# PalamaraLab/FastSMC

Hardware: AMD Instinct MI355X
Metric: haplotype-pairs decoded/sec (whole node) + GB/s vs HBM roofline, 69-state HMM (higher is better)
Workload: dtype f32; 1 GPU; synthetic 1000 haplotypes x 50000 sites, K=69, all 499500 pairs per GPU, FastSMC-mode IBD + posterior-mean/MAP ages, no hashing; mode=ibd, resident_waves=2048, n_cu=256, chunk_sites=512, chunks_per_window=98, resident_chunks=24, beta_stride=2, kernel_member=69, record_gather=none, lib_hash=6c32ac588c314776

## Files before the change

### fastsmc_amd/csrc/fsmc_capi.hip

```cpp
#include <hip/hip_runtime.h>

#include <algorithm>
#include <chrono>
#include <cmath>
#include <cstdio>
#include <cstdlib>
#include <cstring>
#include <new>
#include <string>
#include <type_traits>
#include <vector>

#include "fsmc_identify.h"
#include "fsmc_instances.h"
#include "fsmc_pair_bins.h"
#include "fsmc_pair_cdf.h"
#include "fsmc_pair_tail.h"
#include "fsmc_pair_minima.h"
#include "fsmc_pair_posteriors.h"

namespace fsmc
{
hipError_t idSortCandidates(hipStream_t stream, const fsmc_candidate* in, fsmc_candidate* sorted, unsigned n,
                            unsigned nHaps, unsigned nWords);
hipError_t idSeedDepths(hipStream_t stream, const unsigned long long* words, unsigned nHaps, unsigned nWords,
                        unsigned maxSeeds, unsigned readAhead, unsigned char* depthOut,
                        unsigned hapStride);
}

using namespace fsmc;

namespace fsmc
{
__global__ void add_planes_in_order_kernel(const float* __restrict__ planes, float* __restrict__ acc, size_t n,
                                           int nPlanes, size_t planeStride)
{
  for (size_t i = (size_t)blockIdx.x * blockDim.x + threadIdx.x; i < n; i += (size_t)gridDim.x * blockDim.x) {
    float s = acc[i];
    for (int sl = 0; sl < nPlanes; ++sl) {
      s = s + planes[(size_t)sl * planeStride + i];
    }
    acc[i] = s;
  }
}
}

namespace
{
thread_local std::string g_createError;

struct DevBuf {
  void* p = nullptr;
  size_t bytes = 0;
};

constexpr int kChunkPoolDefault = -1;
constexpr uint32_t kChunkPoolPhiDefault = 200;

enum PairSlicing {
  kSlicePosteriors,
  kSliceMinima,
  kSliceBins,
  kSliceCdf,
  kSliceTail,
  kSliceLoglik,
  kSliceViterbi,
  kPairSlicings
};
}

struct fsmc_ctx {
  int device = 0;
  hipStream_t stream = nullptr;
  bool ownStream = false;
  int nCU = 0;
  uint64_t hbmBytes = 0;
  uint64_t wsLimit = 0;
  double wsEarned = 0;
  double wsAnnounced = 0;
  double wsAnnouncedCredit = 0;
  std::string err;

  unsigned long long* dHaps = nullptr;
  uint32_t nHaps = 0, nSites = 0, W = 0;

  fsmc_pair* dPairs = nullptr;
  fsmc_group* dGroups = nullptr;
  size_t nPairs = 0, nGroups = 0;
  std::vector<fsmc_pair> hPairs;
  std::vector<fsmc_group> hGroups;

  unsigned* dCounters = nullptr;
  unsigned long long* dPhase = nullptr;
  DevBuf ws;
  DevBuf recs;
  size_t recCap = 0;
  DevBuf aux;
  DevBuf out;

  hipEvent_t ev0 = nullptr, ev1 = nullptr;
  bool timed = false;
  int lastSlots = 0;
  int lastChunk = 0, lastMaxChunks = 0, lastResident = 0;
  int residentChunks = -1;
  int chunkPool = kChunkPoolDefault;
  uint32_t chunkPoolPhi = kChunkPoolPhiDefault;
  DevBuf poolState;
  uint32_t lastPoolBuffers = 0;
  uint32_t chunkSites = 0;
  uint32_t betaStride = 0;
  int lastStride = 1;
  bool lastSpsLds = false;
  int lastMember = 0;

  struct IbdQueues {
    uint64_t serial = 0;
    uint64_t maxLen = 0;
    uint64_t maxLenAlone = 0;
    uint32_t pairing = 0;
    bool valid = false;
    bool dual = false;
    bool reordered = false;
    bool alone = false;
    std::vector<fsmc_group> items, unions, rest;
  } q;
  uint64_t worklistSerial = 0;
  fsmc_group* dItems = nullptr;
  fsmc_group* dRest = nullptr;
  uint32_t pairing = 1;
  int lastItems = 0;
  unsigned twoWaves = 0;
  int lastWavesPerWindow = 1;
  hipStream_t side = nullptr;
  hipEvent_t evFork = nullptr, evJoin = nullptr;
  DevBuf wsSide;

  struct {
    uint32_t groups = 0;
    int last = 0;
  } pairSlices[kPairSlicings];
  DevBuf ppStage;
  DevBuf ppRows;
  DevBuf ppAcc;
  hipStream_t copyStream = nullptr;
  void* ppPinned[2] = {nullptr, nullptr};
  size_t ppPinnedBytes = 0;
  hipEvent_t evRows = nullptr, evCopied[2] = {nullptr, nullptr};
  DevBuf pmAcc;
  DevBuf pbAcc;
  DevBuf pcSpec;
  DevBuf plAcc;
  DevBuf pvAcc;
  DevBuf ptAcc;

  DevBuf idStash;
  size_t idStashCount = 0;

  const fsmc_model* ibdModel = nullptr;
  uint32_t ibdFlags = 0;
  bool ibdPending = false;
};

struct fsmc_model {
  fsmc_ctx* ctx = nullptr;
  int K = 0, KP = 0, S = 0, nRows = 0;
  int w2NW = 0;
  float *pi = nullptr, *cR = nullptr, *expT = nullptr;
  float *D = nullptr, *B = nullptr, *U = nullptr, *RR = nullptr;
  float* rowSets = nullptr;
  float* ghostMask = nullptr;
  int* stepRow = nullptr;
  bool sequence = false;
  int *rowGapF = nullptr, *rowSiteB = nullptr, *rowGapB = nullptr;
  float4* emis3 = nullptr;
  unsigned stateThr = 0, ageThr = 0;
  float probThr = 0.f;
};

namespace
{

std::vector<std::string> mappedHipRuntimes()
{
  std::vector<std::string> found;
  if (FILE* f = std::fopen("/proc/self/maps", "r")) {
    char line[4096];
    while (std::fgets(line, sizeof(line), f)) {
      const char* slash = std::strchr(line, '/');
      if (!slash || !std::strstr(slash, "libamdhip64.so")) {
        continue;
// ... 563 lines not shown
    if (ctx->chunkSites) {
      cMin = std::min<size_t>(ctx->chunkSites, L);
    }
    slots = std::min<size_t>(slots, (size_t)(budget.hard / slotBytes(cMin)));
    if (slots == 0) {
      why = "workspace limit too small for the back-pointers of one wave";
      return FSMC_ENOMEM;
    }
    if (ctx->chunkSites) {
      C = cMin;
    } else {
      const uint64_t room = L <= 512 ? budget.hard : budget.soft;
      while (C > cMin && (uint64_t)slots * slotBytes(C) > room) {
        C = std::max(cMin, (C + 1) / 2);
      }
    }
    bytes = slotBytes(C);
  }
  plan = LaunchPlan();
  plan.k = k;
  plan.chunk = (int)C;
  plan.chunkRows = (int)C;
  plan.maxChunks = (int)((L + C - 1) / C);
  plan.wsSlot = bytes / sizeof(float4);
  plan.slots = (int)slots;
  plan.wavesPerWindow = 1;
  plan.bytes = bytes * slots;
  return FSMC_OK;
}

bool twoWavesWanted(const fsmc_ctx* ctx, const KernelChoice& k2, size_t nItems)
{
  if (ctx->twoWaves == 1 || nItems == 0 || !k2.fn) {
    return false;
  }
  if (const char* v = std::getenv("FSMC_DIAG_TWO_WAVE_WINDOWS")) {
    if (std::strcmp(v, "never") == 0) {
      return false;
    }
  }
  int perCU = 0;
  return workgroupsPerCU(k2, 4, 2, perCU) == hipSuccess && perCU >= 1 && nItems <= (size_t)ctx->nCU * perCU;
}

bool planTwoWaves(const fsmc_ctx* ctx, const KernelChoice& k2, size_t nItems, const WsBudget& budget, LaunchPlan& plan)
{
  size_t L = 1;
  for (const fsmc_group& g : ctx->hGroups) {
    L = std::max<size_t>(L, g.to - g.from);
  }
  const size_t K4 = (size_t)(k2.member + 3) / 4;
  plan = LaunchPlan();
  plan.k = k2;
  plan.chunk = (int)L;
  plan.chunkRows = (int)L;
  plan.maxChunks = 1;
  plan.wsSlot = L * K4 * kWave;
  plan.slots = (int)nItems;
  plan.wavesPerWindow = 2;
  plan.bytes = plan.wsSlot * sizeof(float4) * nItems;
  return plan.bytes <= budget.hard && (plan.bytes <= budget.soft || L <= 512);
}

int holdWorkspace(fsmc_ctx* ctx, DevBuf& buf, size_t bytes)
{
  const char* most = std::getenv("FSMC_DIAG_WS_ALLOC_MAX");
  if (most && bytes > std::strtoull(most, nullptr, 10) && !(buf.p && buf.bytes >= bytes)) {
    if (buf.p) {
      (void)hipFree(buf.p);
    }
    buf = DevBuf();
    return fail(ctx, FSMC_ENOMEM, "workspace of " + std::to_string(bytes) + " bytes refused (FSMC_DIAG_WS_ALLOC_MAX)");
  }
  const size_t held = buf.bytes;
  const int rc = ensure(ctx, buf, bytes);
  if (rc != FSMC_OK) {
    (void)hipGetLastError();
  } else if (buf.bytes != held) {
    payForWorkspace(ctx, buf.bytes);
  }
  return rc;
}

int planAndHold(fsmc_ctx* ctx, const fsmc_model* m, int mode, const KernelChoice& k, const std::vector<fsmc_group>& list,
                bool paired, unsigned share, DevBuf& buf, LaunchPlan& plan)
{
  std::string why;
  const int rc = planOneWave(ctx, m, mode, k, list, paired, workspaceBudget(ctx, buf), share, plan, why);
  if (rc != FSMC_OK) {
    return fail(ctx, rc, why);
  }
  if (plan.poolBuffers) {
    FSMC_TRY(ensure(ctx, ctx->poolState, (kPoolClaims + (size_t)plan.poolBuffers) * sizeof(unsigned)));
  }
  return holdWorkspace(ctx, buf, plan.bytes);
}

void recordLaunch(fsmc_ctx* ctx, const KernelChoice& k, const LaunchPlan& plan, int slotsBeside = 0)
{
  ctx->lastMember = k.member;
  ctx->lastStride = k.stride;
  ctx->lastChunk = plan.chunk;
  ctx->lastMaxChunks = plan.maxChunks;
  ctx->lastResident = plan.residentChunks;
  ctx->lastPoolBuffers = plan.poolBuffers;
  ctx->lastWavesPerWindow = plan.wavesPerWindow;
  ctx->lastSlots = plan.slots + slotsBeside;
}

int checkReady(fsmc_ctx* ctx, const fsmc_model* m)
{
  if (!ctx || !m) {
    return fail(ctx, FSMC_EINVAL, "null context or model");
  }
  if (m->ctx != ctx) {
    return fail(ctx, FSMC_EINVAL, "model belongs to another context");
  }
  if (!ctx->dHaps) {
    return fail(ctx, FSMC_ESTATE, "no haplotypes uploaded (fsmc_haps_upload)");
  }
  if (!ctx->dPairs || !ctx->dGroups || ctx->nGroups == 0) {
    return fail(ctx, FSMC_ESTATE, "no work list uploaded (fsmc_worklist_upload)");
  }
  if ((uint32_t)m->S != ctx->nSites) {
    return fail(ctx, FSMC_EINVAL, "model has " + std::to_string(m->S) + " sites but haplotypes have " +
                                      std::to_string(ctx->nSites));
  }
  for (const fsmc_pair& pr : ctx->hPairs) {
    if (pr.hap_a >= ctx->nHaps || pr.hap_b >= ctx->nHaps) {
      return fail(ctx, FSMC_EINVAL, "pair refers to a haplotype row outside the uploaded matrix");
    }
  }
  for (const fsmc_group& g : ctx->hGroups) {
    if (g.to > (uint32_t)m->S) {
      return fail(ctx, FSMC_EINVAL, "group window exceeds the number of sites");
    }
  }
  if (m->K > kMaxStatesAny) {
    return fail(ctx, FSMC_EUNSUPPORTED, "more than " + std::to_string(kMaxStatesAny) + " states");
  }
  return FSMC_OK;
}

void fillParams(const fsmc_ctx* ctx, const fsmc_model* m, const LaunchPlan& plan, uint32_t flags, KParams& p)
{
  std::memset(&p, 0, sizeof(p));
  p.K = m->K;
  p.KP = m->KP;
  p.S = m->S;
  p.W = (int)ctx->W;
  p.nGroups = (int)ctx->nGroups;
  p.chunk = plan.chunk;
  p.chunkRows = plan.chunkRows;
  p.maxChunks = plan.maxChunks;
  p.residentChunks = plan.residentChunks;
  p.flags = flags;
  p.pi = m->pi;
  p.cR = m->cR;
  p.expT = m->expT;
  p.D = m->D;
  p.B = m->B;
  p.U = m->U;
  p.rowSets = m->rowSets;
  p.RR = m->RR;
  p.ghostMask = m->ghostMask;
  p.stepRow = m->stepRow;
  p.rowGapF = m->rowGapF;
  p.rowSiteB = m->rowSiteB;
  p.rowGapB = m->rowGapB;
  p.emis3 = m->emis3;
  p.haps = ctx->dHaps;
  p.pairs = ctx->dPairs;
  p.groups = ctx->dGroups;
  p.counters = ctx->dCounters;
  p.phaseCycles = ctx->dPhase;
  p.ws = (float4*)ctx->ws.p;
  p.wsSlot = plan.wsSlot;
  p.stateThr = m->stateThr;
  p.ageThr = m->ageThr;
  p.spsLds = 0u;
  p.thr[0] = 1000 * m->probThr;
  p.thr[1] = 100 * m->probThr;
  p.thr[2] = 10 * m->probThr;
  p.thr[3] = m->probThr;
  p.recs = (fsmc_ibd_record*)ctx->recs.p;
  p.recCap = (unsigned)ctx->recCap;
}

int checkWorkspace(fsmc_ctx* ctx, const KParams& p, int slots)
{
  const DevBuf& buf = p.ws == (float4*)ctx->wsSide.p ? ctx->wsSide : ctx->ws;
  if (!p.ws || p.ws != (float4*)buf.p || slots < 1 || buf.bytes / sizeof(float4) / (size_t)slots < p.wsSlot) {
    return fail(ctx, FSMC_ESTATE, "the workspace does not hold the launch planned for it");
  }
  return FSMC_OK;
}

int poolParams(fsmc_ctx* ctx, const KernelChoice& k, const KParams& p, const LaunchPlan& plan, int slots, KParamsPool& pp)
{
  static_cast<KParams&>(pp) = p;
  pp.poolOff = plan.poolOff;
  pp.poolBuffers = plan.poolBuffers;
  pp.poolCap = plan.poolCap;
  pp.poolState = (unsigned*)ctx->poolState.p;
  const DevBuf& buf = p.ws == (float4*)ctx->wsSide.p ? ctx->wsSide : ctx->ws;
  const size_t rowF4 = (size_t)((p.K + 3) / 4) * kWave;
  const size_t poolF4 = (size_t)pp.poolBuffers * (size_t)p.chunkRows * rowF4;
  if (!k.poolFn || pp.poolOff < p.wsSlot * (size_t)slots || buf.bytes / sizeof(float4) < pp.poolOff ||
      buf.bytes / sizeof(float4) - pp.poolOff < poolF4 || !pp.poolState ||
      ctx->poolState.bytes / sizeof(unsigned) < kPoolClaims + (size_t)pp.poolBuffers || pp.poolCap < 1 ||
      pp.poolCap > p.maxChunks) {
    return fail(ctx, FSMC_ESTATE, "the workspace does not hold the chunk pool planned for it");
  }
  return FSMC_OK;
}

int resetPool(fsmc_ctx* ctx, const KParamsPool& pp)
{
  FSMC_HIP(ctx, hipMemsetAsync(pp.poolState, 0, (kPoolClaims + (size_t)pp.poolBuffers) * sizeof(unsigned), ctx->stream));
  return FSMC_OK;
}

int launch(fsmc_ctx* ctx, const KernelChoice& k, const KParams& p, int slots, size_t dynLds = 0, bool continues = false,
           const LaunchPlan* plan = nullptr)
{
  if (checkWorkspace(ctx, p, slots) != FSMC_OK) {
    return FSMC_ESTATE;
  }
  const bool pool = plan && plan->poolBuffers != 0;
  KParamsPool pp;
  if (pool) {
    FSMC_TRY(poolParams(ctx, k, p, *plan, slots, pp));
  }
  FSMC_HIP(ctx, hipMemsetAsync(ctx->dCounters, 0, 4 * sizeof(unsigned), ctx->stream));
  if (pool) {
    FSMC_TRY(resetPool(ctx, pp));
  }
  if (!continues) {
    FSMC_HIP(ctx, hipEventRecord(ctx->ev0, ctx->stream));
  }
  if (pool) {
    hipLaunchKernelGGL(k.poolFn, dim3((unsigned)slots), dim3(k.threads), dynLds, ctx->stream, pp);
  } else {
    hipLaunchKernelGGL(k.fn, dim3((unsigned)slots), dim3(k.threads), dynLds, ctx->stream, p);
  }
  FSMC_HIP(ctx, hipGetLastError());
  FSMC_HIP(ctx, hipEventRecord(ctx->ev1, ctx->stream));
  ctx->timed = true;
  return FSMC_OK;
}

int launchBeside(fsmc_ctx* ctx, const KernelChoice& kSide, KParams& pSide, int slotsSide, const LaunchPlan& planSide,
                 const KernelChoice& kMain, KParams& pMain, int slotsMain)
{
  if (checkWorkspace(ctx, pSide, slotsSide) != FSMC_OK || checkWorkspace(ctx, pMain, slotsMain) != FSMC_OK) {
    return FSMC_ESTATE;
  }
  pMain.groupBase = 0;
  pSide.groupBase = 2;
  const bool pool = planSide.poolBuffers != 0;
  KParamsPool ppSide;
  if (pool) {
    FSMC_TRY(poolParams(ctx, kSide, pSide, planSide, slotsSide, ppSide));
  }
  FSMC_HIP(ctx, hipMemsetAsync(ctx->dCounters, 0, 4 * sizeof(unsigned), ctx->stream));
  if (pool) {
    FSMC_TRY(resetPool(ctx, ppSide));
  }
  FSMC_HIP(ctx, hipEventRecord(ctx->ev0, ctx->stream));
  FSMC_HIP(ctx, hipEventRecord(ctx->evFork, ctx->stream));
  FSMC_HIP(ctx, hipStreamWaitEvent(ctx->side, ctx->evFork, 0));
  if (pool) {
    hipLaunchKernelGGL(kSide.poolFn, dim3((unsigned)slotsSide), dim3(kSide.threads), 0, ctx->side, ppSide);
  } else {
    hipLaunchKernelGGL(kSide.fn, dim3((unsigned)slotsSide), dim3(kSide.threads), 0, ctx->side, pSide);
  }
  FSMC_HIP(ctx, hipGetLastError());
  hipLaunchKernelGGL(kMain.fn, dim3((unsigned)slotsMain), dim3(kMain.threads), 0, ctx->stream, pMain);
  FSMC_HIP(ctx, hipGetLastError());
  FSMC_HIP(ctx, hipEventRecord(ctx->evJoin, ctx->side));
  FSMC_HIP(ctx, hipStreamWaitEvent(ctx->stream, ctx->evJoin, 0));
  FSMC_HIP(ctx, hipEventRecord(ctx->ev1, ctx->stream));
  ctx->timed = true;
  return FSMC_OK;
}

uint64_t stagingLimit(const fsmc_ctx* ctx, uint64_t held, unsigned parts)
{
  uint64_t limit = ctx->wsLimit ? ctx->wsLimit : (uint64_t)(0.25 * (double)ctx->hbmBytes);
  size_t freeB = 0, totalB = 0;
  if (hipMemGetInfo(&freeB, &totalB) == hipSuccess) {
    const uint64_t room = (uint64_t)freeB + held;
    const uint64_t reserve = 2ull << 30;
    limit = std::min<uint64_t>(limit, room > reserve ? (room - reserve) / parts : 0);
  }
  return limit;
}

int ensureRowCopies(fsmc_ctx* ctx, size_t need)
{
  if (ctx->ppPinnedBytes < need) {
    for (int i = 0; i < 2; ++i) {
// ... 322 lines not shown
  }
  fsmc_ctx* ctx = new (std::nothrow) fsmc_ctx();
  if (!ctx) {
    return fail(nullptr, FSMC_ENOMEM, "host allocation failed");
  }
  ctx->device = device_id;
  e = hipSetDevice(device_id);
  hipDeviceProp_t prop;
  if (e == hipSuccess) {
    e = hipGetDeviceProperties(&prop, device_id);
  }
  if (e != hipSuccess) {
    delete ctx;
    return fail(nullptr, FSMC_ENODEVICE, std::string("hipSetDevice/hipGetDeviceProperties: ") + hipGetErrorString(e));
  }
  if (std::strncmp(prop.gcnArchName, "gfx950", 6) != 0) {
    std::string arch = prop.gcnArchName;
    delete ctx;
    return fail(nullptr, FSMC_ENODEVICE, "device is " + arch + "; this library is built for gfx950 (MI355X) only");
  }
  ctx->nCU = prop.multiProcessorCount;
  ctx->hbmBytes = (uint64_t)prop.totalGlobalMem;
  if (stream) {
    ctx->stream = (hipStream_t)stream;
  } else {
    e = hipStreamCreateWithFlags(&ctx->stream, hipStreamNonBlocking);
    ctx->ownStream = (e == hipSuccess);
  }
  if (e == hipSuccess) e = hipEventCreate(&ctx->ev0);
  if (e == hipSuccess) e = hipEventCreate(&ctx->ev1);
  if (e == hipSuccess) e = hipStreamCreateWithFlags(&ctx->side, hipStreamNonBlocking);
  if (e == hipSuccess) e = hipEventCreateWithFlags(&ctx->evFork, hipEventDisableTiming);
  if (e == hipSuccess) e = hipEventCreateWithFlags(&ctx->evJoin, hipEventDisableTiming);
  if (e == hipSuccess) e = hipMalloc((void**)&ctx->dCounters, 4 * sizeof(unsigned));
  if (e == hipSuccess) e = hipMalloc((void**)&ctx->dPhase, kPhaseSlots * sizeof(unsigned long long));
  if (e == hipSuccess) e = hipMemset(ctx->dPhase, 0, kPhaseSlots * sizeof(unsigned long long));
  if (e != hipSuccess) {
    std::string msg = std::string("context set-up failed: ") + hipGetErrorString(e);
    fsmc_ctx_destroy(ctx);
    return fail(nullptr, FSMC_EHIP, msg);
  }
  {
    int blocks = 0;
    const hipError_t pe = hipOccupancyMaxActiveBlocksPerMultiprocessor(
      &blocks, decode_kernel<128, kModeIbd, true, false, false>, kWave, 0);
    if (pe != hipSuccess) {
      (void)hipGetLastError();
      const std::vector<std::string> rts = mappedHipRuntimes();
      std::string msg = std::string("kernels of this library cannot be launched (") + hipGetErrorString(pe) + ")";
      int code = FSMC_EHIP;
      if (rts.size() > 1) {
        code = FSMC_ERUNTIME;
        msg += ": two HIP runtimes are loaded in this process (";
        for (size_t i = 0; i < rts.size(); ++i) {
          msg += (i ? ", " : "") + rts[i];
        }
        msg += "): load one libamdhip64 only -- e.g. import torch before this library so that both resolve to the "
               "copy torch bundles, or link both against the same ROCm";
      }
      fsmc_ctx_destroy(ctx);
      return fail(nullptr, code, msg);
    }
  }
  *out = ctx;
  return FSMC_OK;
}

void fsmc_ctx_destroy(fsmc_ctx* ctx)
{
  if (!ctx) {
    return;
  }
  (void)hipSetDevice(ctx->device);
  if (ctx->stream) {
    (void)hipStreamSynchronize(ctx->stream);
  }
  if (ctx->dHaps) (void)hipFree(ctx->dHaps);
  if (ctx->dPairs) (void)hipFree(ctx->dPairs);
  if (ctx->dGroups) (void)hipFree(ctx->dGroups);
  if (ctx->dItems) (void)hipFree(ctx->dItems);
  if (ctx->dRest) (void)hipFree(ctx->dRest);
  if (ctx->dCounters) (void)hipFree(ctx->dCounters);
  if (ctx->poolState.p) (void)hipFree(ctx->poolState.p);
  if (ctx->dPhase) (void)hipFree(ctx->dPhase);
  if (ctx->idStash.p) (void)hipFree(ctx->idStash.p);
  if (ctx->ws.p) (void)hipFree(ctx->ws.p);
  if (ctx->recs.p) (void)hipFree(ctx->recs.p);
  if (ctx->aux.p) (void)hipFree(ctx->aux.p);
  if (ctx->out.p) (void)hipFree(ctx->out.p);
  if (ctx->ev0) (void)hipEventDestroy(ctx->ev0);
  if (ctx->ev1) (void)hipEventDestroy(ctx->ev1);
  if (ctx->evFork) (void)hipEventDestroy(ctx->evFork);
  if (ctx->evJoin) (void)hipEventDestroy(ctx->evJoin);
  if (ctx->side) (void)hipStreamDestroy(ctx->side);
  if (ctx->wsSide.p) (void)hipFree(ctx->wsSide.p);
  if (ctx->copyStream) (void)hipStreamSynchronize(ctx->copyStream);
  if (ctx->ppStage.p) (void)hipFree(ctx->ppStage.p);
  if (ctx->ppRows.p) (void)hipFree(ctx->ppRows.p);
  if (ctx->pcSpec.p) (void)hipFree(ctx->pcSpec.p);
  if (ctx->ptAcc.p) (void)hipFree(ctx->ptAcc.p);
  if (ctx->ppAcc.p) (void)hipFree(ctx->ppAcc.p);
  if (ctx->pmAcc.p) (void)hipFree(ctx->pmAcc.p);
  if (ctx->pbAcc.p) (void)hipFree(ctx->pbAcc.p);
  if (ctx->plAcc.p) (void)hipFree(ctx->plAcc.p);
  if (ctx->pvAcc.p) (void)hipFree(ctx->pvAcc.p);
  for (int i = 0; i < 2; ++i) {
    if (ctx->ppPinned[i]) (void)hipHostFree(ctx->ppPinned[i]);
    if (ctx->evCopied[i]) (void)hipEventDestroy(ctx->evCopied[i]);
  }
  if (ctx->evRows) (void)hipEventDestroy(ctx->evRows);
  if (ctx->copyStream) (void)hipStreamDestroy(ctx->copyStream);
  if (ctx->ownStream && ctx->stream) (void)hipStreamDestroy(ctx->stream);
  delete ctx;
}

int fsmc_ctx_info(const fsmc_ctx* ctx, int32_t* n_cu, int32_t* n_slots, uint64_t* hbm_bytes)
{
  if (!ctx) {
    return FSMC_EINVAL;
  }
  if (n_cu) *n_cu = ctx->nCU;
  if (n_slots) *n_slots = ctx->lastSlots;
  if (hbm_bytes) *hbm_bytes = ctx->hbmBytes;
  return FSMC_OK;
}

int fsmc_ctx_set_workspace_limit(fsmc_ctx* ctx, uint64_t bytes)
{
  if (!ctx) {
    return FSMC_EINVAL;
  }
  ctx->wsLimit = bytes;
  return FSMC_OK;
}

int fsmc_ctx_expect_work(fsmc_ctx* ctx, double pair_sites, int32_t states)
{
  if (!ctx) {
    return fail(nullptr, FSMC_EINVAL, "null context");
  }
  if (!(pair_sites >= 0) || states < 1) {
    return fail(ctx, FSMC_EINVAL, "expected work: pair-sites >= 0 and states >= 1");
  }
  if (pair_sites == 0) {
    ctx->wsEarned = std::max(0.0, ctx->wsEarned - ctx->wsAnnouncedCredit);
    ctx->wsAnnounced = 0;
    ctx->wsAnnouncedCredit = 0;
    return FSMC_OK;
  }
  const double seconds = pair_sites * (8.0 * states + 0.25) / (0.8 * 8e12);
  const double credit = std::min(earnScale() * kEarnFraction * seconds * kAllocBytesPerSecond,
                                 std::max(0.0, (double)ctx->hbmBytes - ctx->wsAnnouncedCredit));
  ctx->wsAnnounced += seconds;
  ctx->wsAnnouncedCredit += credit;
  ctx->wsEarned += credit;
  return FSMC_OK;
}

int fsmc_ctx_set_chunk_sites(fsmc_ctx* ctx, uint32_t sites)
{
  if (!ctx) {
    return FSMC_EINVAL;
  }
  ctx->chunkSites = sites;
  return FSMC_OK;
}

int fsmc_ctx_set_beta_stride(fsmc_ctx* ctx, uint32_t stride)
{
  if (!ctx || stride > 2) {
    return fail(ctx, FSMC_EINVAL, "beta stride must be 0 (automatic), 1 or 2");
  }
  ctx->betaStride = stride;
  return FSMC_OK;
}

int fsmc_ctx_last_beta_stride(const fsmc_ctx* ctx, int32_t* stride)
{
  if (!ctx || !stride) {
    return FSMC_EINVAL;
  }
  *stride = ctx->lastStride;
  return FSMC_OK;
}

int fsmc_ctx_last_plan(const fsmc_ctx* ctx, int32_t* chunk_sites, int32_t* max_chunks, int32_t* n_slots)
{
  if (!ctx) {
    return FSMC_EINVAL;
  }
  if (chunk_sites) *chunk_sites = ctx->lastChunk;
  if (max_chunks) *max_chunks = ctx->lastMaxChunks;
  if (n_slots) *n_slots = ctx->lastSlots;
  return FSMC_OK;
}

int fsmc_ctx_set_resident_chunks(fsmc_ctx* ctx, int32_t chunks)
{
  if (!ctx || chunks < -1) {
    return fail(ctx, FSMC_EINVAL, "resident chunks: -1 (automatic), 0 (none) or a count");
  }
  ctx->residentChunks = chunks;
  return FSMC_OK;
}

int fsmc_ctx_last_resident_chunks(const fsmc_ctx* ctx, int32_t* chunks)
{
  if (!ctx || !chunks) {
    return FSMC_EINVAL;
  }
  *chunks = ctx->lastResident;
  return FSMC_OK;
}

int fsmc_ctx_set_chunk_pool(fsmc_ctx* ctx, int32_t mode, uint32_t phi_percent)
{
  if (!ctx || mode < -1 || mode > 1) {
    return fail(ctx, FSMC_EINVAL, "chunk pool: -1 (automatic), 0 (never) or 1 (also in launches of one or two rounds and the sums)");
  }
  if (phi_percent != 0 && (phi_percent < 100 || phi_percent > 100000)) {
    return fail(ctx, FSMC_EINVAL, "chunk pool: phi is 100 ... 100000 per cent of a wave's share (0: the default)");
  }
  ctx->chunkPool = mode;
  ctx->chunkPoolPhi = phi_percent ? phi_percent : kChunkPoolPhiDefault;
  return FSMC_OK;
}

int fsmc_ctx_last_chunk_pool(fsmc_ctx* ctx, uint32_t* buffers, uint32_t* kept, uint32_t* rebuilt, uint32_t* outstanding)
{
  if (!ctx) {
    return FSMC_EINVAL;
  }
  uint32_t k = 0, r = 0, o = 0;
  if (ctx->lastPoolBuffers) {
    FSMC_HIP(ctx, hipSetDevice(ctx->device));
    FSMC_HIP(ctx, hipStreamSynchronize(ctx->stream));
    std::vector<unsigned> st(kPoolClaims + (size_t)ctx->lastPoolBuffers);
    if (!ctx->poolState.p || ctx->poolState.bytes < st.size() * sizeof(unsigned)) {
      return fail(ctx, FSMC_ESTATE, "the chunk pool's state is gone");
    }
    FSMC_HIP(ctx, hipMemcpy(st.data(), ctx->poolState.p, st.size() * sizeof(unsigned), hipMemcpyDeviceToHost));
    k = st[kPoolKept];
    r = st[kPoolRebuilt];
    for (size_t i = kPoolClaims; i < st.size(); ++i) {
      o += st[i] != 0u;
    }
  }
  if (buffers) *buffers = ctx->lastPoolBuffers;
  if (kept) *kept = k;
  if (rebuilt) *rebuilt = r;
  if (outstanding) *outstanding = o;
  return FSMC_OK;
}

int fsmc_ctx_set_pair_posterior_slice(fsmc_ctx* ctx, uint32_t groups) { return setPairSlice(ctx, kSlicePosteriors, groups); }
int fsmc_ctx_last_pair_posterior_slices(const fsmc_ctx* ctx, int32_t* slices) { return lastPairSlices(ctx, kSlicePosteriors, slices); }
int fsmc_ctx_set_pair_minima_slice(fsmc_ctx* ctx, uint32_t groups) { return setPairSlice(ctx, kSliceMinima, groups); }
int fsmc_ctx_last_pair_minima_slices(const fsmc_ctx* ctx, int32_t* slices) { return lastPairSlices(ctx, kSliceMinima, slices); }
int fsmc_ctx_set_pair_bins_slice(fsmc_ctx* ctx, uint32_t groups) { return setPairSlice(ctx, kSliceBins, groups); }
int fsmc_ctx_last_pair_bins_slices(const fsmc_ctx* ctx, int32_t* slices) { return lastPairSlices(ctx, kSliceBins, slices); }
int fsmc_ctx_set_pair_cdf_slice(fsmc_ctx* ctx, uint32_t groups) { return setPairSlice(ctx, kSliceCdf, groups); }
int fsmc_ctx_last_pair_cdf_slices(const fsmc_ctx* ctx, int32_t* slices) { return lastPairSlices(ctx, kSliceCdf, slices); }
int fsmc_ctx_set_pair_tail_slice(fsmc_ctx* ctx, uint32_t groups) { return setPairSlice(ctx, kSliceTail, groups); }
int fsmc_ctx_last_pair_tail_slices(const fsmc_ctx* ctx, int32_t* slices) { return lastPairSlices(ctx, kSliceTail, slices); }
int fsmc_ctx_set_pair_loglik_slice(fsmc_ctx* ctx, uint32_t groups) { return setPairSlice(ctx, kSliceLoglik, groups); }
int fsmc_ctx_last_pair_loglik_slices(const fsmc_ctx* ctx, int32_t* slices) { return lastPairSlices(ctx, kSliceLoglik, slices); }
int fsmc_ctx_set_pair_viterbi_slice(fsmc_ctx* ctx, uint32_t groups) { return setPairSlice(ctx, kSliceViterbi, groups); }
int fsmc_ctx_last_pair_viterbi_slices(const fsmc_ctx* ctx, int32_t* slices) { return lastPairSlices(ctx, kSliceViterbi, slices); }

int fsmc_ctx_last_kernel(const fsmc_ctx* ctx, int32_t* member)
{
  if (!ctx || !member) {
    return FSMC_EINVAL;
  }
  *member = ctx->lastMember;
  return FSMC_OK;
}

int fsmc_model_create(fsmc_ctx* ctx, const fsmc_model_desc* d, fsmc_model** out)
{
  if (!ctx || !d || !out) {
    return fail(ctx, FSMC_EINVAL, "null argument");
  }
  *out = nullptr;
  if (d->K < 2 || d->S < 1 || d->n_rows < 1) {
    return fail(ctx, FSMC_EINVAL, "need K >= 2, S >= 1, n_rows >= 1");
  }
  if (d->K > kMaxStatesAny) {
    return fail(ctx, FSMC_EUNSUPPORTED, "more than " + std::to_string(kMaxStatesAny) + " states");
  }
  if (!d->pi || !d->col_ratios || !d->exp_times || !d->D || !d->B || !d->U || !d->RR || !d->step_row || !d->e1 ||
      !d->e0m1 || !d->e2m0) {
    return fail(ctx, FSMC_EINVAL, "null table pointer in model description");
  }
  if (d->state_threshold > (uint32_t)d->K || d->age_threshold > (uint32_t)d->K) {
    return fail(ctx, FSMC_EINVAL, "state/age threshold larger than K");
  }
  const bool seq = d->sequence != 0;
  if (seq && (!d->gap_row_f || !d->site_row_f || !d->gap_row_b || !d->site_row_b || !d->hom)) {
    return fail(ctx, FSMC_EINVAL, "sequence mode needs gap_row_f, site_row_f, gap_row_b, site_row_b and hom");
  }
  const int32_t* rowArrays[5] = {d->step_row, seq ? d->gap_row_f : nullptr, seq ? d->site_row_f : nullptr,
                                 seq ? d->gap_row_b : nullptr, seq ? d->site_row_b : nullptr};
  static const char* const rowNames[5] = {"step_row", "gap_row_f", "site_row_f", "gap_row_b", "site_row_b"};
  for (int a = 0; a < 5; ++a) {
    for (int32_t s = 1; rowArrays[a] && s < d->S; ++s) {
      if (rowArrays[a][s] < 0 || rowArrays[a][s] >= d->n_rows) {
        return fail(ctx, FSMC_EINVAL,
                    std::string(rowNames[a]) + "[" + std::to_string(s) + "] outside the transition tables");
      }
    }
  }
  FSMC_HIP(ctx, hipSetDevice(ctx->device));
  fsmc_model* m = new (std::nothrow) fsmc_model();
  if (!m) {
    return fail(ctx, FSMC_ENOMEM, "host allocation failed");
  }
  m->ctx = ctx;
  m->K = d->K;
  m->KP = (d->K + kKPad - 1) / kKPad * kKPad;
  if (d->K > 128 && d->K <= kMaxStatesW2) {
    const W2Member w = w2Member(d->K);
    m->w2NW = w.NW;
    m->KP = w.NW * w.KH;
  }
  m->S = d->S;
  m->nRows = d->n_rows;
  m->stateThr = d->state_threshold;
  m->ageThr = d->age_threshold;
// ... 1523 lines not shown
```

### fastsmc_amd/csrc/fsmc_decode_kernel_body.h

```cpp
#if FSMC_DECODE_POOL
template <int KT, int MODE, bool TRACK, bool HALF>
__global__ __launch_bounds__(kWave, minWavesPerSimd(KT)) void decode_kernel_pool(const KParamsPool p)
#else
template <int KT, int MODE, bool TRACK, bool SEQ, bool HALF, bool DUAL = false>
__global__ __launch_bounds__(kWave, minWavesPerSimd(KT)) void decode_kernel(const KParams p)
#endif
{
#if FSMC_DECODE_POOL
  constexpr bool SEQ = false, DUAL = false;
#endif
  static_assert(!HALF || (!SEQ && (MODE == kModeIbd || MODE == kModeSums)),
                "beta stride 2 is built for the array-mode IBD decode and the array-mode sums over pairs");
  static_assert(KT > 0 && KT <= kMaxStates, "a member of the kernel family (fsmc_instances.h)");
  static_assert(!DUAL || (MODE == kModeIbd && !SEQ), "two half-groups per wave: array-mode IBD");
  constexpr bool kRotate = !SEQ;
  constexpr int KA = KT;
  constexpr int K4A = (KA + 3) / 4;
  constexpr int E4A = ((KA + kKPad - 1) / kKPad) * (kKPad / 4);
  constexpr int NC = SEQ ? 4 : 3;
  constexpr int NL = (NC * E4A + kWave - 1) / kWave;
  constexpr int K = KT;
  const int Kreal = kGhost<KT> ? p.K : K;
  constexpr int K4 = (K + 3) >> 2;
  const int KP = p.KP;
// ... 139 lines not shown
          emisLds[q & 1][idx] = r.v[i];
        }
      }
      __builtin_amdgcn_wave_barrier();
    };

    auto stageEmis = [&](const int q) {
      const gchar_p src = uniformPtr(p.emis3 + (size_t)q * (NC * E4));
#pragma unroll
      for (int i = 0; i < NL; ++i) {
        const int idx = lane + i * kWave;
        if (idx < NC * E4) {
          dmaToLds((gf32x4_p)(src + (size_t)i * (kWave * sizeof(float4)) + laneOff), &emisLds[q & 1][i * kWave]);
        }
      }
    };
    RowIndexBlock stepRows;
    auto stepRowOf = [&](const int site) -> int { return stepRows.at(p.stepRow, p.S, lane, site); };
    auto waitEmisRows = [&](const bool storesBehind) {
      constexpr unsigned n = (unsigned)K4A;
      if (storesBehind && n < 64) {
        __builtin_amdgcn_s_waitcnt(0x0F70 | (n & 15u) | ((n >> 4) << 14));
      } else {
        waitVm0();
      }
    };

    float w[KA];
    Diag cycW;
#if defined(FSMC_REGION_STAMPS)
    cycW.last = (unsigned)__builtin_readcyclecounter();
#endif
#if defined(FSMC_PHASE_STAMPS)
    long long cycB = 0, cycR = 0, cycA = 0;
    long long stamp = (long long)clock64();
#define FSMC_STAMP(acc)                                                                                                \
  do {                                                                                                                 \
    const long long now_ = (long long)clock64();                                                                       \
    (acc) += now_ - stamp;                                                                                             \
    stamp = now_;                                                                                                      \
  } while (0)
#else
#define FSMC_STAMP(acc) ((void)0)
#endif

    auto betaGapStep = [&](float (&b)[KA], const int q, const EmisRegs& rows) {
      commitEmis(q, rows);
      const int row = tRowGapB[q];
      beta_step<KT, KA, false, kSeqSyncLoads<SEQ, KT, MODE>>(K, b, w, tabs, row, &emisLds[q & 1][3 * E4], cycW);
    };
    auto betaSeqStep = [&](float (&b)[KA], const int pos) {
      const int q = pos + 1;
      const bool gap = pos > from;
      EmisRegs ev;
      if (gap) {
        ev = prefetchEmis(pos);
      }
      const int c = obsClass(q);
      const int row = tRowSiteB[q];
      beta_step<KT, KA, true, kSeqSyncLoads<SEQ, KT, MODE>>(K, b, w, tabs, row, &emisLds[q & 1][c * E4], cycW);
      if (gap) {
        betaGapStep(b, pos, ev);
      }
    };

    {
      float b[KA];
      if constexpr (!kRotate) {
        beta_init<KT, KA>(K, p.K, b);
      }
      int ckJ = (aEnd < to) ? nChunks : nChunks - 1;
      int ckPos = (aEnd < to) ? aEnd : from + ckJ * C;
#if FSMC_DECODE_POOL
      float4* keep = nullptr;
      auto enterChunk = [&](const int j) {
        if (!pooled) {
          keep = j < nResident ? resBase + (size_t)j * p.chunkRows * vecF4 : nullptr;
          return;
        }
        keep = nullptr;
        if (j < p.poolCap) {
          int got = -1;
          if (lane == 0) {
            for (int t = 0; t < kPoolProbes; ++t) {
              const unsigned c = __hip_atomic_fetch_add(&p.poolState[kPoolCursor], 1u, __ATOMIC_RELAXED,
                                                        __HIP_MEMORY_SCOPE_AGENT) % p.poolBuffers;
              unsigned expected = 0u;
              if (__hip_atomic_compare_exchange_strong(&p.poolState[kPoolClaims + c], &expected, 1u, __ATOMIC_RELAXED,
                                                       __ATOMIC_RELAXED, __HIP_MEMORY_SCOPE_AGENT)) {
                got = (int)c;
                break;
              }
            }
            poolTable[j] = got;
          }
          got = __builtin_amdgcn_readfirstlane(got);
          if (got >= 0) {
            keep = poolBase + (size_t)got * p.chunkRows * vecF4;
          }
        }
      };
      if (!single && ckJ < nChunks) {
        enterChunk(ckJ);
      }
#endif
      auto afterBeta = [&](const int pos) -> bool {
        if (single) {
          const int rel = pos - from;
          if (pos < aEnd && (!HALF || (rel & 1) || pos == aEnd - 1)) {
            store_vec<KT, KA>(K, chunkbuf + slotOf(rel) * vecF4, laneOff, b);
            return true;
          }
        } else {
          bool out = false;
#if FSMC_DECODE_POOL
          if (keep != nullptr) {
#else
          if (kResidentBuilt && ckJ < nResident && pos < aEnd) {
#endif
            const int relc = pos - ckPos;
            const int hiJ = ckPos + C < aEnd ? ckPos + C : aEnd;
            if (!HALF || (relc & 1) || pos == hiJ - 1) {
#if FSMC_DECODE_POOL
              store_vec<KT, KA>(K, keep + slotOf(relc) * vecF4, laneOff, b);
#else
              store_vec<KT, KA>(K, resBase + ((size_t)ckJ * p.chunkRows + slotOf(relc)) * vecF4, laneOff, b);
#endif
              out = true;
            }
          }
          if (__builtin_expect(pos == ckPos && ckJ >= 1, 0)) {
            store_vec<KT, KA>(K, ckpt + (size_t)ckJ * vecF4, laneOff, b);
            ckJ -= 1;
            ckPos = from + ckJ * C;
#if FSMC_DECODE_POOL
            enterChunk(ckJ);
#endif
            out = true;
          }
          return out;
        }
        return false;
      };
      if constexpr (SEQ) {
        if (to - 1 > from) {
          betaGapStep(b, to - 1, prefetchEmis(to - 1));
        }
      }
      if constexpr (!kRotate) {
        afterBeta(to - 1);
      }
      if constexpr (SEQ) {
        for (int pos = to - 2; pos >= from; --pos) {
          betaSeqStep(b, pos);
          afterBeta(pos);
        }
      } else {
        if (to - 2 >= from) {
          stageEmis(to - 1);
        }
        if constexpr (kRotate) {
          float bsum = 0.f;
#pragma unroll
          for (int k = 0; k < K; ++k) {
            w[k] = (!kGhost<KT> || k < p.K) ? 1.0f : 0.f;
            bsum = bsum + w[k];
          }
          const float bsumInit = bsum;
          auto openBeta = [&](const int q) {
            if constexpr (DUAL) {
              if (q == toA - 1 || q == toB - 1) {
                const bool sel = myTo - 1 == q;
#pragma unroll
// ... 583 lines not shown
                    float4 sv[K4];
#pragma unroll
                    for (int g4 = 0; g4 < K4; g4 += kG) {
                      if ((unsigned)(4 * g4) < nAgeL) {
#pragma unroll
                        for (int j = 0; j < kG; ++j) {
                          if (g4 + j < K4) {
                            sv[g4 + j] = loadBlock(g4 + j);
                          }
                        }
                      }
                    }
#pragma unroll
                    for (int g4 = 0; g4 < K4; g4 += kG) {
                      if ((unsigned)(4 * g4) < nAgeL) {
#pragma unroll
                        for (int j = 0; j < kG; ++j) {
                          if (g4 + j < K4) {
                            addBlock(g4 + j, sv[g4 + j]);
                          }
                        }
                      }
                    }
                  } else {
#pragma unroll
                    for (int g4 = 0; g4 < K4; g4 += kG) {
                      if ((unsigned)(4 * g4) >= nAgeL) {
                        break;
                      }
                      float4 sv[kG];
#pragma unroll
                      for (int j = 0; j < kG; ++j) {
                        if (g4 + j < K4) {
                          sv[j] = loadBlock(g4 + j);
                        }
                      }
#pragma unroll
                      for (int j = 0; j < kG; ++j) {
                        if (g4 + j < K4) {
                          addBlock(g4 + j, sv[j]);
                        }
                      }
                    }
                  }
                };
                if constexpr (kSpsLdsBuilt<MODE, SEQ, DUAL>) {
                  if (spsInLds) {
                    rounds(std::true_type{});
                  } else {
                    rounds(std::false_type{});
                  }
                } else {
                  rounds(std::false_type{});
                }
              }
            }
            acc = (level == 4) ? 0.f : (opening ? s : acc + s);
            if (opening) {
              segStart = pos;
            }
            cur = level;
            if constexpr (DUAL) {
              if (__builtin_expect(pos == stA - 1 || pos == stB - 1, 0)) {
                if (pos == myST - 1) {
                  if (valid && cur != 4) {
                    emit(segStart, pos);
                  }
                  cur = 4;
                }
              }
            } else if (__builtin_expect(pos == aEnd - 1, 0)) {
              if (valid && cur != 4) {
                emit(segStart, pos);
              }
            }
          }
        }
        FSMC_END(cycW, 12);
      }
#if FSMC_DECODE_POOL
      if (pooled && resident) {
        waitVm0();
        if (lane == 0) {
          __hip_atomic_exchange(&p.poolState[kPoolClaims + poolBuf], 0u, __ATOMIC_RELEASE, __HIP_MEMORY_SCOPE_AGENT);
          __hip_atomic_fetch_add(&p.poolState[kPoolKept], 1u, __ATOMIC_RELAXED, __HIP_MEMORY_SCOPE_AGENT);
        }
      }
#endif
      FSMC_STAMP(cycA);
    }
#if defined(FSMC_REGION_STAMPS)
    if (lane == 0 && p.phaseCycles) {
#pragma unroll
      for (int r = 0; r < 16; ++r) {
        atomicAdd(&p.phaseCycles[8 + r], (unsigned long long)cycW.acc[r]);
      }
    }
#endif
#if defined(FSMC_DIAG_GROUP_TIMES)
    if (MODE == kModeIbd && lane == 0) {
      const unsigned long long t1 = __builtin_amdgcn_s_memrealtime();
      const unsigned idx = atomicAdd(&p.counters[1], 1u);
      if (idx < p.recCap) {
        fsmc_ibd_record r;
        r.pair = pairIdx;
        r.start = -1;
        r.end = (int)blockIdx.x;
        r.prob = (float)((double)(t1 & 0xFFFFFFFFull) / 1e5);
        r.post_mean = (float)((double)(diagT0 & 0xFFFFFFFFull) / 1e5);
        r.map = __int_as_float((int)(__builtin_amdgcn_s_getreg(63492) & 0xFFFFu) |
                               (int)((__builtin_amdgcn_s_getreg(63508) & 0xFu) << 16));
        p.recs[idx] = r;
      }
    }
#endif
#if defined(FSMC_PHASE_STAMPS)
    if (lane == 0 && p.phaseCycles) {
      atomicAdd(&p.phaseCycles[0], (unsigned long long)cycB);
      atomicAdd(&p.phaseCycles[1], (unsigned long long)cycR);
      atomicAdd(&p.phaseCycles[2], (unsigned long long)cycA);
      atomicAdd(&p.phaseCycles[3], 1ull);
      atomicAdd(&p.phaseCycles[4], (unsigned long long)cycW.waitCycles);
    }
#endif
  }
}
```

### fastsmc_amd/csrc/fsmc_kernels.h

```cpp
#pragma once

#include <hip/hip_runtime.h>

#include <type_traits>

#include "../../include/fastsmc_hip.h"

namespace fsmc
{

constexpr int kWave = 64;

typedef const float __attribute__((address_space(4))) * cfloat_p;
typedef const int __attribute__((address_space(4))) * cint_p;
typedef const unsigned __attribute__((address_space(4))) * cuint_p;
typedef float f32x2 __attribute__((ext_vector_type(2)));
typedef float f32x4 __attribute__((ext_vector_type(4)));
typedef float f32x8 __attribute__((ext_vector_type(8)));
typedef float f32x16 __attribute__((ext_vector_type(16)));
constexpr int kMaxStates = 256;
constexpr int kMaxStatesW2 = 1024;
constexpr int kMaxStatesAny = 4096;

enum Mode : int { kModeIbd = 0, kModeDump = 1, kModePerPair = 2, kModeSums = 3 };

struct KParams {
  int K;
  int KP;
  int S;
  int W;
  int nGroups;
  int groupBase;
  int chunk;
  int chunkRows;
  int maxChunks;
  unsigned flags;
  const float* pi;
  const float* cR;
  const float* expT;
  const float* D;
  const float* B;
  const float* U;
  const float* rowSets;
  const float* RR;
  const float* ghostMask;
  const int* stepRow;
  const int* rowGapF;
  const int* rowSiteB;
  const int* rowGapB;
  const float4* emis3;
  const unsigned long long* haps;
  const fsmc_pair* pairs;
  const fsmc_group* groups;
  unsigned* counters;
  float4* ws;
  size_t wsSlot;
  unsigned stateThr, ageThr;
  unsigned spsLds;
  float thr[4];
  fsmc_ibd_record* recs;
  unsigned recCap;
  float* dumpOut;
  const size_t* dumpOffsets;
  float* ppMean;
  int* ppMap;
  const float* expCoal;
  unsigned long long* phaseCycles;
  float* sums;
  size_t sumsPlane;
  size_t sumsSlot;
  const unsigned* batchFirst;
  int residentChunks;
};
struct KParamsPool : KParams {
  size_t poolOff;
  unsigned poolBuffers;
  int poolCap;
  unsigned* poolState;
};
enum { kPoolCursor = 0, kPoolKept = 1, kPoolRebuilt = 2, kPoolClaims = 4 };
constexpr int kPoolProbes = 4;

#if defined(__HIP_DEVICE_COMPILE__)
#define FSMC_GCN_ASM(...) asm volatile(__VA_ARGS__)
#else
#define FSMC_GCN_ASM(...) ((void)0)
#endif

__device__ __forceinline__ f32x4 sload4(cfloat_p p, const int byteOff)
{
  f32x4 v = {};
  FSMC_GCN_ASM("s_load_dwordx4 %0, %1, %2" : "=s"(v) : "s"(p), "i"(byteOff));
  return v;
}
__device__ __forceinline__ f32x8 sload8(cfloat_p p, const int byteOff)
{
  f32x8 v = {};
#if defined(FSMC_DIAG_NOSMEM)
  FSMC_GCN_ASM("; no load %0 %1 %2" : "=s"(v) : "s"(p), "i"(byteOff));
#else
  FSMC_GCN_ASM("s_load_dwordx8 %0, %1, %2" : "=s"(v) : "s"(p), "i"(byteOff));
#endif
  return v;
}
#if defined(FSMC_NO_TOUCH)
constexpr bool kTouch = false;
#else
constexpr bool kTouch = true;
#endif
struct Touched {
  float r[4];
};
template <int FIRST, int STEP = 16>
__device__ __forceinline__ void touchLines(Touched& t, cfloat_p p, const int firstState)
{
  FSMC_GCN_ASM("s_load_dword %0, %4, %5\n\ts_load_dword %1, %4, %6\n\ts_load_dword %2, %4, %7\n\ts_load_dword %3, %4, %8"
               : "=&s"(t.r[0]), "=&s"(t.r[1]), "=&s"(t.r[2]), "=&s"(t.r[3])
               : "s"(p), "i"((firstState + FIRST * STEP) * 4), "i"((firstState + (FIRST + 1) * STEP) * 4),
                 "i"((firstState + (FIRST + 2) * STEP) * 4), "i"((firstState + (FIRST + 3) * STEP) * 4));
}
__device__ __forceinline__ void holdTouched(Touched& a)
{
  FSMC_GCN_ASM("" : "+s"(a.r[0]), "+s"(a.r[1]), "+s"(a.r[2]), "+s"(a.r[3]));
}
#define FSMC_SWAIT_INSN "s_waitcnt lgkmcnt(0)"
__device__ __forceinline__ void swait(f32x8& a, f32x8& b)
{
  FSMC_GCN_ASM(FSMC_SWAIT_INSN : "+s"(a), "+s"(b));
}
__device__ __forceinline__ void swait(f32x16& a, f32x16& b)
{
  FSMC_GCN_ASM(FSMC_SWAIT_INSN : "+s"(a), "+s"(b));
}
__device__ __forceinline__ void swait(f32x8& a, f32x8& b, f32x8& c, f32x8& d)
{
  FSMC_GCN_ASM(FSMC_SWAIT_INSN : "+s"(a), "+s"(b), "+s"(c), "+s"(d));
}
template <int N> struct SV;
template <> struct SV<4> {
  typedef f32x4 T;
  static __device__ __forceinline__ T loadAt(cfloat_p p, const int firstState) { return sload4(p, firstState * 4); }
};
template <> struct SV<8> {
  typedef f32x8 T;
  static __device__ __forceinline__ T loadAt(cfloat_p p, const int firstState) { return sload8(p, firstState * 4); }
};
template <> struct SV<16> {
  typedef f32x16 T;
  static __device__ __forceinline__ T loadAt(cfloat_p p, const int firstState)
  {
    f32x16 v = {};
#if defined(FSMC_DIAG_NOSMEM)
    FSMC_GCN_ASM("; no load %0 %1 %2" : "=s"(v) : "s"(p), "i"(firstState * 4));
#else
    FSMC_GCN_ASM("s_load_dwordx16 %0, %1, %2" : "=s"(v) : "s"(p), "i"(firstState * 4));
#endif
    return v;
  }
};
__device__ __forceinline__ void swait(f32x4& a, f32x4& b, f32x4& c, f32x4& d)
{
  FSMC_GCN_ASM(FSMC_SWAIT_INSN : "+s"(a), "+s"(b), "+s"(c), "+s"(d));
}

// ... 721 lines not shown
```

Measured before the change: 276,300 pairs/s.

## Replace probe-based chunk-pool claims with a tagged lock-free free-list stack

Swaps the cursor-plus-CAS probing allocator for the chunk-buffer pool with a Treiber stack using a 64-bit tagged head (ABA counter) and per-buffer link words. A pop now always succeeds while any buffer is free, rather than failing after four probes and forcing a rebuild. The pool is reset each launch by copying a prebuilt initial list image instead of a memset, and the default pool size factor rises from 200 to 225. Release pays for an extra fence and CAS retry loop, and the single head word can become a contention point across many waves.

```diff
diff --git a/fastsmc_amd/csrc/fsmc_capi.hip b/fastsmc_amd/csrc/fsmc_capi.hip
--- a/fastsmc_amd/csrc/fsmc_capi.hip
+++ b/fastsmc_amd/csrc/fsmc_capi.hip
@@ -55,7 +55,7 @@
 };
 
 constexpr int kChunkPoolDefault = -1;
-constexpr uint32_t kChunkPoolPhiDefault = 200;
+constexpr uint32_t kChunkPoolPhiDefault = 225;
 
 enum PairSlicing {
   kSlicePosteriors,
@@ -106,6 +106,8 @@
   int chunkPool = kChunkPoolDefault;
   uint32_t chunkPoolPhi = kChunkPoolPhiDefault;
   DevBuf poolState;
+  DevBuf poolInit;
+  uint32_t poolInitBuffers = 0;
   uint32_t lastPoolBuffers = 0;
   uint32_t chunkSites = 0;
   uint32_t betaStride = 0;
@@ -835,6 +837,25 @@
   return rc;
 }
 
+int holdPoolState(fsmc_ctx* ctx, uint32_t buffers)
+{
+  const size_t words = poolWords(buffers);
+  FSMC_TRY(ensure(ctx, ctx->poolState, words * sizeof(unsigned)));
+  if (ctx->poolInit.p && ctx->poolInitBuffers == buffers) {
+    return FSMC_OK;
+  }
+  ctx->poolInitBuffers = 0;
+  FSMC_TRY(ensure(ctx, ctx->poolInit, words * sizeof(unsigned)));
+  std::vector<unsigned> img(words, 0u);
+  img[kPoolHead] = 1u;
+  for (uint32_t i = 0; i < buffers; ++i) {
+    img[kPoolLinks + i] = i + 1 < buffers ? i + 2u : 0u;
+  }
+  FSMC_HIP(ctx, hipMemcpy(ctx->poolInit.p, img.data(), words * sizeof(unsigned), hipMemcpyHostToDevice));
+  ctx->poolInitBuffers = buffers;
+  return FSMC_OK;
+}
+
 int planAndHold(fsmc_ctx* ctx, const fsmc_model* m, int mode, const KernelChoice& k, const std::vector<fsmc_group>& list,
                 bool paired, unsigned share, DevBuf& buf, LaunchPlan& plan)
 {
@@ -844,7 +865,7 @@
     return fail(ctx, rc, why);
   }
   if (plan.poolBuffers) {
-    FSMC_TRY(ensure(ctx, ctx->poolState, (kPoolClaims + (size_t)plan.poolBuffers) * sizeof(unsigned)));
+    FSMC_TRY(holdPoolState(ctx, plan.poolBuffers));
   }
   return holdWorkspace(ctx, buf, plan.bytes);
 }
@@ -961,7 +982,8 @@
   const size_t poolF4 = (size_t)pp.poolBuffers * (size_t)p.chunkRows * rowF4;
   if (!k.poolFn || pp.poolOff < p.wsSlot * (size_t)slots || buf.bytes / sizeof(float4) < pp.poolOff ||
       buf.bytes / sizeof(float4) - pp.poolOff < poolF4 || !pp.poolState ||
-      ctx->poolState.bytes / sizeof(unsigned) < kPoolClaims + (size_t)pp.poolBuffers || pp.poolCap < 1 ||
+      ctx->poolState.bytes / sizeof(unsigned) < poolWords(pp.poolBuffers) ||
+      ctx->poolInitBuffers != pp.poolBuffers || pp.poolCap < 1 ||
       pp.poolCap > p.maxChunks) {
     return fail(ctx, FSMC_ESTATE, "the workspace does not hold the chunk pool planned for it");
   }
@@ -970,7 +992,8 @@
 
 int resetPool(fsmc_ctx* ctx, const KParamsPool& pp)
 {
-  FSMC_HIP(ctx, hipMemsetAsync(pp.poolState, 0, (kPoolClaims + (size_t)pp.poolBuffers) * sizeof(unsigned), ctx->stream));
+  FSMC_HIP(ctx, hipMemcpyAsync(pp.poolState, ctx->poolInit.p, poolWords(pp.poolBuffers) * sizeof(unsigned),
+                               hipMemcpyDeviceToDevice, ctx->stream));
   return FSMC_OK;
 }
 
@@ -1459,6 +1482,7 @@
   if (ctx->dRest) (void)hipFree(ctx->dRest);
   if (ctx->dCounters) (void)hipFree(ctx->dCounters);
   if (ctx->poolState.p) (void)hipFree(ctx->poolState.p);
+  if (ctx->poolInit.p) (void)hipFree(ctx->poolInit.p);
   if (ctx->dPhase) (void)hipFree(ctx->dPhase);
   if (ctx->idStash.p) (void)hipFree(ctx->idStash.p);
   if (ctx->ws.p) (void)hipFree(ctx->ws.p);
@@ -1612,16 +1636,19 @@
   if (ctx->lastPoolBuffers) {
     FSMC_HIP(ctx, hipSetDevice(ctx->device));
     FSMC_HIP(ctx, hipStreamSynchronize(ctx->stream));
-    std::vector<unsigned> st(kPoolClaims + (size_t)ctx->lastPoolBuffers);
+    std::vector<unsigned> st(poolWords(ctx->lastPoolBuffers));
     if (!ctx->poolState.p || ctx->poolState.bytes < st.size() * sizeof(unsigned)) {
       return fail(ctx, FSMC_ESTATE, "the chunk pool's state is gone");
     }
     FSMC_HIP(ctx, hipMemcpy(st.data(), ctx->poolState.p, st.size() * sizeof(unsigned), hipMemcpyDeviceToHost));
     k = st[kPoolKept];
     r = st[kPoolRebuilt];
-    for (size_t i = kPoolClaims; i < st.size(); ++i) {
-      o += st[i] != 0u;
-    }
+    size_t freeBuffers = 0;
+    for (unsigned at = st[kPoolHead]; at != 0u && freeBuffers <= ctx->lastPoolBuffers;
+         at = at <= ctx->lastPoolBuffers ? st[kPoolLinks + at - 1] : 0u) {
+      ++freeBuffers;
+    }
+    o = freeBuffers <= ctx->lastPoolBuffers ? ctx->lastPoolBuffers - (uint32_t)freeBuffers : ctx->lastPoolBuffers;
   }
   if (buffers) *buffers = ctx->lastPoolBuffers;
   if (kept) *kept = k;
diff --git a/fastsmc_amd/csrc/fsmc_decode_kernel_body.h b/fastsmc_amd/csrc/fsmc_decode_kernel_body.h
--- a/fastsmc_amd/csrc/fsmc_decode_kernel_body.h
+++ b/fastsmc_amd/csrc/fsmc_decode_kernel_body.h
@@ -245,13 +245,16 @@
         if (j < p.poolCap) {
           int got = -1;
           if (lane == 0) {
-            for (int t = 0; t < kPoolProbes; ++t) {
-              const unsigned c = __hip_atomic_fetch_add(&p.poolState[kPoolCursor], 1u, __ATOMIC_RELAXED,
-                                                        __HIP_MEMORY_SCOPE_AGENT) % p.poolBuffers;
-              unsigned expected = 0u;
-              if (__hip_atomic_compare_exchange_strong(&p.poolState[kPoolClaims + c], &expected, 1u, __ATOMIC_RELAXED,
-                                                       __ATOMIC_RELAXED, __HIP_MEMORY_SCOPE_AGENT)) {
-                got = (int)c;
+            unsigned long long* const poolHead = reinterpret_cast<unsigned long long*>(p.poolState + kPoolHead);
+            unsigned* const poolLink = p.poolState + kPoolLinks;
+            unsigned long long head = __hip_atomic_load(poolHead, __ATOMIC_RELAXED, __HIP_MEMORY_SCOPE_AGENT);
+            while ((unsigned)head != 0u) {
+              const unsigned top = (unsigned)head - 1u;
+              const unsigned below = __hip_atomic_load(&poolLink[top], __ATOMIC_RELAXED, __HIP_MEMORY_SCOPE_AGENT);
+              const unsigned long long popped = (((head >> 32) + 1ull) << 32) | below;
+              if (__hip_atomic_compare_exchange_strong(poolHead, &head, popped, __ATOMIC_RELAXED, __ATOMIC_RELAXED,
+                                                       __HIP_MEMORY_SCOPE_AGENT)) {
+                got = (int)top;
                 break;
               }
             }
@@ -1001,7 +1004,22 @@
       if (pooled && resident) {
         waitVm0();
         if (lane == 0) {
-          __hip_atomic_exchange(&p.poolState[kPoolClaims + poolBuf], 0u, __ATOMIC_RELEASE, __HIP_MEMORY_SCOPE_AGENT);
+#if !defined(FSMC_DIAG_POOL_RELAXED)
+          __builtin_amdgcn_fence(__ATOMIC_RELEASE, "agent");
+          waitVm0();
+#endif
+          unsigned long long* const poolHead = reinterpret_cast<unsigned long long*>(p.poolState + kPoolHead);
+          unsigned* const poolLink = p.poolState + kPoolLinks;
+          unsigned long long head = __hip_atomic_load(poolHead, __ATOMIC_RELAXED, __HIP_MEMORY_SCOPE_AGENT);
+          for (;;) {
+            __hip_atomic_store(&poolLink[poolBuf], (unsigned)head, __ATOMIC_RELAXED, __HIP_MEMORY_SCOPE_AGENT);
+            waitVm0();
+            const unsigned long long pushed = (((head >> 32) + 1ull) << 32) | (unsigned)(poolBuf + 1);
+            if (__hip_atomic_compare_exchange_strong(poolHead, &head, pushed, __ATOMIC_RELAXED, __ATOMIC_RELAXED,
+                                                     __HIP_MEMORY_SCOPE_AGENT)) {
+              break;
+            }
+          }
           __hip_atomic_fetch_add(&p.poolState[kPoolKept], 1u, __ATOMIC_RELAXED, __HIP_MEMORY_SCOPE_AGENT);
         }
       }
diff --git a/fastsmc_amd/csrc/fsmc_kernels.h b/fastsmc_amd/csrc/fsmc_kernels.h
--- a/fastsmc_amd/csrc/fsmc_kernels.h
+++ b/fastsmc_amd/csrc/fsmc_kernels.h
@@ -78,8 +78,8 @@
   int poolCap;
   unsigned* poolState;
 };
-enum { kPoolCursor = 0, kPoolKept = 1, kPoolRebuilt = 2, kPoolClaims = 4 };
-constexpr int kPoolProbes = 4;
+enum { kPoolKept = 1, kPoolRebuilt = 2, kPoolHead = 32, kPoolLinks = 64 };
+constexpr size_t poolWords(const unsigned buffers) { return kPoolLinks + (size_t)buffers; }
 
 #if defined(__HIP_DEVICE_COMPILE__)
 #define FSMC_GCN_ASM(...) asm volatile(__VA_ARGS__)
```

Measured after the change: 277,600 pairs/s, median of 6. Within noise of the previous version (+0.5%).
